# EnverRamirez/KiD

Hardware: AMD Instinct MI355X
Metric: thompson_mp_column_steps_per_sec (higher is better)
Workload: dtype f64; 1 GPU; config3: 100000 perturbed mixed-phase deep-convection columns, nz=120, dt=10 s, fp64; ncol_per_gpu=100000, nz=120

## Files before the change

### kid_amd/csrc/thompson_column.hip

```cpp
#include <hip/hip_runtime.h>

#include "thompson_column.h"
#include "fastmath.h"
#include "thompson_consts_gen.h"
#include "kernel_src_hash.h"

#include <cstdlib>
#include <type_traits>

#if defined(KIDMP_PROFILING)
#define DBGSTOP (a.debug_stop)
#define DBGCLK(var) const long long var = (DBGSTOP == 7 || DBGSTOP == 8) ? (long long)__builtin_readcyclecounter() : 0
#define PSTOP(code, expr)
#elif defined(KIDMP_PSTOP_AT)
#define DBGSTOP KIDMP_PSTOP_AT
#define DBGCLK(var)
#define PSTOP(code, expr) if (DBGSTOP == (code)) { L(V_QFAC, k) = (expr); break; }
#else
#define DBGSTOP 0
#define DBGCLK(var)
#define PSTOP(code, expr)
#endif

#ifndef KIDMP_REAL
// ... 374 lines not shown
            }
    }
}

__device__ inline real nr_from_mvd(real rr, real mvd)
{
    const dreal lamr = (R_(3.0) + mu_r + R_(0.672)) / Q(mvd);
    return real(R_(kc::crg[1]) * R_(kc::org3) * rr * cube(lamr) / am_r);
}

template <char SPECIES>
__device__ inline real eff_aero(real D, real Da, real visc, real rhoa, real Temp)
{
    const real boltzman = R_(1.3806503E-23), meanPath = R_(0.0256E-6);
    real vt;
    if constexpr (SPECIES == 'r')
        vt = -R_(0.1021) + R_(4.932E3) * D - R_(0.9551E6) * D * D + R_(0.07934E9) * D * D * D - R_(0.002362E12) * D * D * D * D;
    else if constexpr (SPECIES == 's')
        vt = av_s * fpow(D, bv_s);
    else
        vt = av_g * fpow(D, bv_g);
    const real Cc = R_(1.) + R_(2.) * meanPath / Q(Da) * (R_(1.257) + R_(0.4) * fm::exp(-R_(0.55) * Da / meanPath));
    const real diff = boltzman * Temp * Cc / Q((R_(3.) * PI * visc * Da));
    const real Re = R_(0.5) * rhoa * D * vt / Q(visc);
    const real Sc_ = visc / Q((rhoa * diff));
    const real St = Da * Da * vt * R_(1000.) / Q((R_(9.) * visc * D));
    const real aval = R_(1.) + fm::log(R_(1.) + Re);
    const real St2 = (R_(1.2) + R_(1.) / R_(12.) * aval) / Q((R_(1.) + aval));
    const real sRe = fm::sqrt_pos(Re);
    real Eff = R_(4.) / Q((Re * Sc_)) * (R_(1.) + R_(0.4) * sRe * fpow(Sc_, R_(0.3333)) + R_(0.16) * sRe * fm::sqrt_pos(Sc_))
             + R_(4.) * Da / Q(D) * (R_(0.02) + Da / Q(D) * (R_(1.) + R_(2.) * sRe));
    if (St > St2) {
        const real x = (St - St2) / Q((St - St2 + R_(0.666667)));
        Eff = Eff + x * fm::sqrt_pos(x);
    }
    return fmax(R_(1.E-5), fmin(Eff, R_(1.0)));
}
__device__ inline real ice_demott(real tempc, real rho, real nifa)
{
    const real rho_not0 = R_(101325.) / (R_(287.05) * R_(273.15));
    const real nifa_cc = nifa * rho_not0 * R_(1.E-6) / Q(rho);
    real xni = (R_(5.94e-5) * fpow(-tempc, R_(3.33))) * fpow(nifa_cc, ((-R_(0.0264) * (tempc)) + R_(0.0033)));
    xni = xni * rho / rho_not0 * R_(1000.);
    return fmax(R_(0.), xni);
}
__device__ inline real ice_koop(real temp, real qv, real qvs, real naero, real DT)
{
    const real R_uni = R_(8.314), ar_volume = R_(4.) / R_(3.) * PI * (R_(2.5e-6) * R_(2.5e-6) * R_(2.5e-6));
    const real satw = qv / Q(qvs);
    const real mu_diff = R_(210368.0) + (R_(131.438) * temp) - (R_(3.32373E6) / Q(temp)) - (R_(41729.1) * fm::log(temp));
    const real a_w_i = fm::exp(mu_diff / Q((R_uni * temp)));
    const real delta_aw = satw - a_w_i;
    real log_J_rate = -R_(906.7) + (R_(8502.0) * delta_aw) - (R_(26924.0) * delta_aw * delta_aw) + (R_(29180.0) * delta_aw * delta_aw * delta_aw);
    log_J_rate = fmin(R_(20.0), log_J_rate);
    const real J_rate = fm::exp10(fmax(log_J_rate, -R_(30.)));
    const real prob_h = fmin(R_(1.) - fm::exp(fmax(-J_rate * ar_volume * DT, -R_(80.))), R_(1.));
    real xni = R_(0.);
    if (prob_h > R_(0.)) xni = fmin(prob_h * naero, R_(1000.E3));
    return fmax(R_(0.0), xni);
}
__device__ inline real activ_ncloud(real Ww, real NCCN)
{
    const real ta_Na[7] = {R_(10.0), R_(31.6), R_(100.0), R_(316.0), R_(1000.0), R_(3160.0), R_(10000.0)};
    const real ta_Ww[9] = {R_(0.01), R_(0.0316), R_(0.1), R_(0.316), R_(1.0), R_(3.16), R_(10.0), R_(31.6), R_(100.0)};
    real n_local = NCCN * R_(1.E-6), w_local = Ww;
    if (n_local >= ta_Na[6]) n_local = ta_Na[6] - R_(1.0);
    else if (n_local <= ta_Na[0]) n_local = ta_Na[0] + R_(1.0);
    real xa = ta_Na[0], xb = ta_Na[1];
#pragma unroll
    for (int n = 1; n < 7; ++n) if (n_local >= ta_Na[n - 1] && n_local < ta_Na[n]) { xa = ta_Na[n - 1]; xb = ta_Na[n]; }
    if (w_local >= ta_Ww[8]) w_local = ta_Ww[8] - R_(1.0);
    else if (w_local <= ta_Ww[0]) w_local = ta_Ww[0] + R_(0.001);
    real ya = ta_Ww[0], yb = ta_Ww[1];
#pragma unroll
    for (int n = 1; n < 9; ++n) if (w_local >= ta_Ww[n - 1] && w_local < ta_Ww[n]) { ya = ta_Ww[n - 1]; yb = ta_Ww[n]; }
    const real x1 = fm::log(xa), x2 = fm::log(xb), y1 = fm::log(ya), y2 = fm::log(yb);
    const real nx = fm::log(n_local), wy = fm::log(w_local);
    const real t = (nx - x1) / Q((x2 - x1)), u = (wy - y1) / Q((y2 - y1));
    const real fraction = (R_(1.0) - t) * (R_(1.0) - u) * R_(1.0) + t * (R_(1.0) - u) * R_(1.0) + t * u * R_(1.0) + (R_(1.0) - t) * u * R_(1.0);
    return NCCN * fraction;
}

enum Slot {
    V_TEMP = 0, V_QV, V_RHO, V_RC, V_RI , V_RR, V_RS , V_RG , V_NI , V_NR, V_QVSI , V_SSATW,
    V_SSATI , V_N0X , V_PRES, V_NWFA , V_NIFA , V_NCRAW , V_NIRAW , V_NRRAW ,
    V_TTEN = 32 , V_QFAC, V_QCTEN , V_NCTEN , V_QITEN, V_NITEN, V_QRTEN, V_NRTEN, V_QSTEN, V_QGTEN,
    V_RHO2 , V_BOOST , V_RHOK , V_RR2, V_NR2, V_VTS0 ,
    V_MVDK ,
    NSLOT_V = 64,
    NSLOT_MIXED = 13,
    NSLOT_WARM = 10
};

enum Flag { F_QC = 1, F_QI = 2, F_QR = 4, F_QS = 8, F_QG = 16 };

struct SlotMap { int v[NSLOT_V]; };
constexpr SlotMap make_map(bool warm)
{
    SlotMap m{};
    for (int i = 0; i < NSLOT_V; ++i) m.v[i] = -1;
    if (warm) {
        m.v[V_TEMP] = 0; m.v[V_QV] = 1; m.v[V_RHO] = 2; m.v[V_RC] = 3; m.v[V_SSATW] = 4; m.v[V_RR] = 5; m.v[V_PRES] = 6; m.v[V_NR] = 7;
        m.v[V_QCTEN] = 0; m.v[V_NCTEN] = 1; m.v[V_QITEN] = 2; m.v[V_NITEN] = 3; m.v[V_QRTEN] = 4; m.v[V_NRTEN] = 5;
        m.v[V_QSTEN] = 6; m.v[V_QGTEN] = 7; m.v[V_RR2] = 8; m.v[V_NR2] = 9;
    } else {
        m.v[V_TEMP] = 0; m.v[V_QV] = 1; m.v[V_RHO] = 2; m.v[V_RC] = 3; m.v[V_RR] = 4; m.v[V_NI] = 5; m.v[V_NR] = 6;
        m.v[V_QVSI] = 7; m.v[V_SSATW] = 8; m.v[V_SSATI] = 9; m.v[V_N0X] = 10; m.v[V_PRES] = 11; m.v[V_RI] = 12;
        m.v[V_QFAC] = 0; m.v[V_QITEN] = 1; m.v[V_NITEN] = 2; m.v[V_QRTEN] = 3; m.v[V_NRTEN] = 4; m.v[V_QSTEN] = 5;
        m.v[V_QGTEN] = 6; m.v[V_BOOST] = 7; m.v[V_RHOK] = 8; m.v[V_RR2] = 9; m.v[V_MVDK] = 10; m.v[V_NR2] = 11; m.v[V_VTS0] = 12;
    }
    return m;
}
constexpr SlotMap WMAP = make_map(true), MMAP = make_map(false);
__device__ constexpr int mixed_slot(int v) { return MMAP.v[v]; }
template <bool WARM, int S>
__device__ constexpr int slot_of()
{
    static_assert(S >= 0 && S < NSLOT_V, "no such slot");
    static_assert((WARM ? WMAP.v[S] : MMAP.v[S]) >= 0, "this slot is not staged in this layout");
    return WARM ? WMAP.v[S] : MMAP.v[S];
}

}

__constant__ Consts g_consts[MAX_CONST_SLOTS];

typedef __attribute__((address_space(1))) real greal;
typedef __attribute__((address_space(1))) double grate;
__device__ inline greal *uniform_ptr(const real *p)
{
    const unsigned long long v = reinterpret_cast<unsigned long long>(p);
    const unsigned lo = __builtin_amdgcn_readfirstlane(unsigned(v));
    const unsigned hi = __builtin_amdgcn_readfirstlane(unsigned(v >> 32));
    return (greal *)((static_cast<unsigned long long>(hi) << 32) | lo);
}

__device__ inline greal *gptr(const real *p, int64_t off)
{
    return (greal *)reinterpret_cast<unsigned long long>(p) + off;
}
__device__ inline grate *gptr_rate(const double *p, int64_t off)
{
    return (grate *)reinterpret_cast<unsigned long long>(p) + off;
}

typedef const __attribute__((address_space(4))) StepArgs CArgs;
__device__ inline CArgs *kargs()
{
    CArgs *p = (CArgs *)__builtin_amdgcn_kernarg_segment_ptr();
    asm volatile("" : "+s"(p));
    return p;
}

#ifndef KIDMP_MIXED_WAVES
#define KIDMP_MIXED_WAVES 3
#endif
#ifndef KIDMP_WARM_WAVES
#define KIDMP_WARM_WAVES 4
#endif
#ifdef KIDMP_NUM_VGPR
#define KIDMP_VGPR_ATTR __attribute__((amdgpu_num_vgpr(KIDMP_NUM_VGPR)))
#else
#define KIDMP_VGPR_ATTR
#endif
template <int NJ, int NL, int CPW, bool RATES, bool WARM, bool AERO, bool NCCOL = false>
__global__ __launch_bounds__(CPW *WAVE, WARM ? KIDMP_WARM_WAVES : ((RATES || AERO) ? 2 : KIDMP_MIXED_WAVES)) KIDMP_VGPR_ATTR void thompson_column_step(const StepArgs a)
{
    constexpr int BL = WAVE / CPW;
    __shared__ dreal Lsh[CPW][(WARM ? NSLOT_WARM : NSLOT_MIXED) * NL];
    __shared__ int s_alive[CPW];
    __shared__ int s_next;
    __shared__ real s_cc[7][16];
    __shared__ double s_p10[P10_N];
    __shared__ real s_ntc[NCCOL && CPW > 1 ? CPW : 1];
    static_assert(!(NCCOL && AERO), "a per-column droplet number is for non-aerosol contexts");
    const int wv = CPW > 1 ? __builtin_amdgcn_readfirstlane(int(threadIdx.x) / WAVE) : 0;
    dreal *const Lw = Lsh[wv];
#define L(slot, k) Lw[slot_of<WARM, slot>() * NL + (k)]
#define LR(slot, k) Lw[mixed_slot(slot) * NL + (k)]

#if KFM_TABLES
    constexpr bool TABLES_AT_ENTRY = sizeof(dreal) == 8 && (!WARM || REAL_IS_BINARY32), TABLES_LATE = sizeof(dreal) == 8 && !TABLES_AT_ENTRY;
    if constexpr (TABLES_AT_ENTRY) {
        fm::tab::load_tables(int(threadIdx.x), CPW * WAVE);
        __syncthreads();
    }
    fm::tab::TableRequest<CPW * WAVE> mathtab;
    if constexpr (TABLES_LATE) mathtab.request(int(threadIdx.x));
#endif
    const Consts &c = g_consts[a.cslot];
    const int lane = lane_id();
    const int nz = a.nz;
    __builtin_assume(nz >= 2 && nz <= 4 * WAVE);
    const int kte = nz - 1;
    const unsigned nzu = unsigned(nz), kteu = unsigned(kte);
    constexpr bool iiwarm = WARM;
    const real DT = a.dt;
    const real odt = frcp(DT), odts = frcp(DT);
    real Nt_c = c.Nt_c;
    constexpr int NTAB = WARM ? 112 : 112 + P10_N;
    static_assert(P10_N == 32, "Consts::lds_tab holds 32 powers of ten");
    constexpr int TPT = (NTAB + CPW * WAVE - 1) / (CPW * WAVE);
    double tabv[TPT];
#pragma unroll
    for (int i = 0; i < TPT; ++i) {
        const int t = int(threadIdx.x) + i * CPW * WAVE;
        tabv[i] = c.lds_tab[t < NTAB ? t : 0];
    }

    const int64_t col0 = int64_t(blockIdx.x) * CPW;
    const int64_t col = col0 + wv;
    bool alive = col < a.ncol;
    if constexpr (NCCOL) {
        if (alive) {
            const unsigned long long pv = reinterpret_cast<unsigned long long>(kargs()->set_nc_col);
            const unsigned lo = __builtin_amdgcn_readfirstlane(unsigned(pv)), hi = __builtin_amdgcn_readfirstlane(unsigned(pv >> 32));
            typedef __attribute__((address_space(1))) double gdouble;
            Nt_c = real(((const gdouble *)((static_cast<unsigned long long>(hi) << 32) | lo))[col] * 1.e6);
        }
    }
    {
        if (DBGSTOP == 9) return;
        DBGCLK(clk0);
        const int64_t base = col * int64_t(nz), base0 = col0 * int64_t(nz);
        int pst[NJ];
        real mvdB[NJ], rgB[NJ];
        bool any_micro = false;
        bool col_frozen = true;
#pragma unroll
        for (int j = 0; j < NJ; ++j) { pst[j] = 0; mvdB[j] = R_(0.); rgB[j] = R1; }
        if (alive) {
        real i_t[NJ], i_qv[NJ], i_p[NJ], i_qc[NJ], i_qi[NJ], i_qr[NJ], i_qs[NJ], i_qg[NJ], i_ni[NJ], i_nr[NJ];
        real i_nc[NJ], i_nwfa[NJ], i_nifa[NJ];
        {
        CArgs *ka = kargs();
        const greal *gt = gptr(ka->t, base), *gqv = gptr(ka->qv, base), *gp = gptr(ka->p, base),
                      *gqc = gptr(ka->qc, base), *gqi = gptr(ka->qi, base), *gqr = gptr(ka->qr, base),
                      *gqs = gptr(ka->qs, base), *gqg = gptr(ka->qg, base), *gni = gptr(ka->ni, base),
                      *gnr = gptr(ka->nr, base), *gnc = gptr(ka->nc, base), *gnwfa = gptr(ka->nwfa, base),
                      *gnifa = gptr(ka->nifa, base);
#pragma unroll
        for (int j = 0; j < NJ; ++j) {
            const unsigned k = unsigned(lane) + unsigned(WAVE) * unsigned(j);
            const unsigned kc = k < nzu ? k : kteu;
            i_t[j] = gt[kc];   i_qv[j] = gqv[kc]; i_p[j] = gp[kc];   i_qc[j] = gqc[kc]; i_qi[j] = gqi[kc];
            i_qr[j] = gqr[kc]; i_qs[j] = gqs[kc]; i_qg[j] = gqg[kc]; i_ni[j] = gni[kc]; i_nr[j] = gnr[kc];
            i_nc[j] = gnc[kc]; i_nwfa[j] = gnwfa[kc]; i_nifa[j] = gnifa[kc];
        }
        }
        if constexpr (iiwarm) {
            bool fz = false;
#pragma unroll
            for (int j = 0; j < NJ; ++j) fz = fz || i_qi[j] != R_(0.) || i_qs[j] != R_(0.) || i_qg[j] != R_(0.) || i_ni[j] != R_(0.);
            col_frozen = __any(fz);
        }
#pragma unroll
        for (int j = 0; j < NJ; ++j) {
            const unsigned k = unsigned(lane) + unsigned(WAVE) * unsigned(j);
            pst[j] = 0; mvdB[j] = R_(0.); rgB[j] = R1;
            if (k >= nzu) continue;
            const real temp = i_t[j];
            const real qv = fmax(R_(1.E-10), i_qv[j]);
            const real pres = i_p[j];
            const real rho = R_(0.622) * pres / Q((Rgas * temp * (qv + R_(0.622))));
            const real qc1 = i_qc[j], qi1 = i_qi[j], qr1 = i_qr[j], qs1 = i_qs[j], qg1 = i_qg[j];
            int f = 0;
            real ri = R1, ni = R2, rr = R1, nr = R2, rg = R1;

            if (qc1 > R1) {
                f |= F_QC;
            }
            if (qi1 > R1) {
                f |= F_QI;
                ri = qi1 * rho;
                ni = fmax(R2, i_ni[j] * rho);
                if (ni <= R2) {
                    const dreal lami = R_(kc::cie[1]) / R_(25.E-6);
                    ni = fmin(R_(499.e3), R_(kc::cig[0]) * R_(kc::oig2) * ri / am_i * cube(lami));
                }
                dreal lami = root3(am_i * R_(kc::cig[1]) * R_(kc::oig1) * ni / Q(ri));
                const real xDi = (bm_i + mu_i + R_(1.)) * (frcp(lami));
                if (xDi < R_(5.E-6)) {
                    lami = R_(kc::cie[1]) / R_(5.E-6);
                    ni = fmin(R_(499.e3), R_(kc::cig[0]) * R_(kc::oig2) * ri / am_i * cube(lami));
                } else if (xDi > R_(300.E-6)) {
                    lami = R_(kc::cie[1]) / R_(300.E-6);
                    ni = R_(kc::cig[0]) * R_(kc::oig2) * ri / am_i * cube(lami);
                }
            }
            if (qr1 > R1) {
                f |= F_QR;
                rr = qr1 * rho;
                nr = fmax(R2, i_nr[j] * rho);
                if (nr <= R2) nr = nr_from_mvd(rr, R_(1.0E-3));
                const dreal lamr = root3(am_r * R_(kc::crg[2]) * R_(kc::org2) * nr / Q(rr));
                real mvd = (R_(3.0) + mu_r + R_(0.672)) / Q(lamr);
                if (mvd > R_(2.5E-3)) {
                    mvd = R_(2.5E-3);
                    nr = nr_from_mvd(rr, mvd);
                } else if (mvd < D0r * R_(0.75)) {
                    mvd = D0r * R_(0.75);
                    nr = nr_from_mvd(rr, mvd);
                }
                mvdB[j] = mvd;
            }
            if (qs1 > R1) f |= F_QS;
            if (qg1 > R1) { f |= F_QG; rg = qg1 * rho; }
            rgB[j] = rg;

            const real tempc = temp - R_(273.15);
            const real qvs = rslf(pres, temp);
            const real qvsi = tempc <= R_(0.0) ? rsif(pres, temp) : qvs;
            real ssatw = qv / Q(qvs) - R_(1.);
            real ssati = qv / Q(qvsi) - R_(1.);
            if (fabs(ssatw) < eps) ssatw = R_(0.0);
            if (fabs(ssati) < eps) ssati = R_(0.0);
            if (f != 0 || ssati > R_(0.0)) any_micro = true;
            pst[j] = f | (temp >= R_(270.65) ? 1 << 16 : 0);

            L(V_TEMP, k) = temp;  L(V_QV, k) = i_qv[j];   L(V_RHO, k) = rho;
            L(V_RC, k) = (f & F_QC) ? qc1 : R_(0.);  L(V_RR, k) = (f & F_QR) ? qr1 : R_(0.);
            L(V_NR, k) = nr;      L(V_SSATW, k) = ssatw;
            L(V_PRES, k) = pres;
            if constexpr (!iiwarm) {
                L(V_RI, k) = (f & F_QI) ? qi1 : R_(0.);
                L(V_NI, k) = ni;      L(V_QVSI, k) = qvsi;  L(V_SSATI, k) = ssati;
            }
        }

        if (!__any(any_micro)) {
            CArgs *ka = kargs();
            greal *gqc = gptr(ka->qc, base), *gnc = gptr(ka->nc, base), *gqi = gptr(ka->qi, base),
                    *gni = gptr(ka->ni, base), *gqr = gptr(ka->qr, base), *gnr = gptr(ka->nr, base),
                    *gqs = gptr(ka->qs, base), *gqg = gptr(ka->qg, base);
            grate *grates = RATES ? gptr_rate(ka->rates, col * int64_t(KIDMP_NRATES_) * nz) : nullptr;
#pragma unroll
            for (int j = 0; j < NJ; ++j) {
                const unsigned k = unsigned(lane) + unsigned(WAVE) * unsigned(j);
                if (k >= nzu) continue;
                gqc[k] = R_(0.0); gnc[k] = R_(0.0);
                gqr[k] = R_(0.0); gnr[k] = R_(0.0);
                if (col_frozen) { gqi[k] = R_(0.0); gni[k] = R_(0.0); gqs[k] = R_(0.0); gqg[k] = R_(0.0); }
                if (RATES)
                    for (int r = 0; r < KIDMP_NRATES_; ++r) grates[int64_t(r) * nz + k] = R_(0.);
            }
            if (ka->nstep && lane < 4) ka->nstep[col * 4 + lane] = 0;
            alive = false;
        }

        if constexpr (!iiwarm) if (alive) {
            int k0l = 0;
#pragma unroll
            for (int j = 0; j < NJ; ++j)
                if (pst[j] >> 16) k0l = lane + WAVE * j;
            const int k_0 = wave_max_i(k0l);
            dreal n0[NJ];
            bool in_[NJ], ur_[NJ];
#pragma unroll
            for (int j = 0; j < NJ; ++j) {
                const unsigned k = unsigned(lane) + unsigned(WAVE) * unsigned(j);
                in_[j] = k < nzu;
                ur_[j] = int(k) > k_0 && (pst[j] & F_QR) && mvdB[j] > R_(100.E-6);
            }
            graupel_N0_column<NJ>(in_, ur_, mvdB, rgB, dreal(c.n0g_empty), n0);
            suffix_min<NJ>(n0);
#pragma unroll
            for (int j = 0; j < NJ; ++j) {
                const unsigned k = unsigned(lane) + unsigned(WAVE) * unsigned(j);
                if (k < nzu) L(V_N0X, k) = n0[j];
            }
        }

        }
        if (DBGSTOP == 1) { if (alive && lane == 0) kargs()->ppt[col * 4] += Lw[0] + Lw[9 * NL + 1]; return; }
#pragma unroll
        for (int i = 0; i < TPT; ++i) {
            const int t = int(threadIdx.x) + i * CPW * WAVE;
            if (t < 112) s_cc[t >> 4][t & 15] = real(tabv[i]);
            else if (!WARM && t < NTAB) s_p10[t - 112] = tabv[i];
        }
#if KFM_TABLES
        if constexpr (TABLES_LATE) mathtab.store(int(threadIdx.x));
#endif
        DBGCLK(clk1);
        if (CPW > 1) {
            if (lane == 0) s_alive[wv] = alive ? (col_frozen ? 3 : 1) : 0;
            if (threadIdx.x == 0) s_next = 0;
            if constexpr (NCCOL) if (lane == 0) s_ntc[wv] = Nt_c;
            __syncthreads();
        }
        DBGCLK(clk2);
        if (CPW == 1 && !alive) return;
#undef L
#define L(slot, k) Lp[slot_of<WARM, slot>() * NL + (k)]
        const int nband = (nz + BL - 1) / BL;
#pragma unroll 1
        for (int it = 0;; ++it) {
            int seq = it;
            if (CPW > 1) {
                int t = 0;
                if (lane == 0) t = atomicAdd(&s_next, 1);
                seq = __builtin_amdgcn_readfirstlane(t);
            }
            if (seq >= nband) break;
            const int band = CPW > 1 ? (nband - 1) / 2 + ((seq & 1) ? (seq + 1) / 2 : -(seq / 2)) : seq;
            const int cw = CPW > 1 ? lane / BL : 0;
            const unsigned k = unsigned(band * BL) + unsigned(lane % BL);
            if (k < nzu && (CPW == 1 || s_alive[cw])) do {
            dreal *const Lp = Lsh[cw];
            if constexpr (NCCOL && CPW > 1) Nt_c = s_ntc[cw];
            const unsigned gk = unsigned(cw) * nzu + k;
            CArgs *ka1 = kargs();
            real qi1c, qs1c, qg1c, ni_b = R2, ni1_raw, qvsi = R_(0.), ssati = R_(0.), diffu = R_(0.);
            const bool frozen_here = !iiwarm || (CPW == 1 ? col_frozen : (s_alive[cw] & 2) != 0);
            if constexpr (iiwarm) {
                qi1c = R_(0.); qs1c = R_(0.); qg1c = R_(0.); ni1_raw = R_(0.);
                if (frozen_here) {
                    const real rqi = gptr(ka1->qi, base0)[gk], rqs = gptr(ka1->qs, base0)[gk], rqg = gptr(ka1->qg, base0)[gk];
                    ni1_raw = gptr(ka1->ni, base0)[gk];
                    qi1c = rqi > R1 ? rqi : R_(0.);  qs1c = rqs > R1 ? rqs : R_(0.);  qg1c = rqg > R1 ? rqg : R_(0.);
                }
            } else {
                const real rqs = gptr(ka1->qs, base0)[gk], rqg = gptr(ka1->qg, base0)[gk];
                qi1c = L(V_RI, k);  qs1c = rqs > R1 ? rqs : R_(0.);  qg1c = rqg > R1 ? rqg : R_(0.);
                ni_b = L(V_NI, k);
                qvsi = L(V_QVSI, k);  ssati = L(V_SSATI, k);
            }
            real nwfa_in = R_(0.), nifa_in = R_(0.), nc_in = R_(0.), nr_in = R_(0.);
            if constexpr (AERO) {
                nwfa_in = gptr(ka1->nwfa, base0)[gk]; nifa_in = gptr(ka1->nifa, base0)[gk];
                nc_in = gptr(ka1->nc, base0)[gk];     nr_in = gptr(ka1->nr, base0)[gk];
                if constexpr (!iiwarm) ni1_raw = gptr(ka1->ni, base0)[gk];
            }
            const bool L_qc = L(V_RC, k) > R_(0.), L_qi = qi1c > R_(0.), L_qr = L(V_RR, k) > R_(0.), L_qs = qs1c > R_(0.), L_qg = qg1c > R_(0.);
            const real pres = L(V_PRES, k);
            grate *grates = RATES ? gptr_rate(ka1->rates, col0 * int64_t(KIDMP_NRATES_) * nz) + int64_t(cw) * KIDMP_NRATES_ * nz : nullptr;
            const real temp = L(V_TEMP, k), qv_raw = L(V_QV, k), rho = L(V_RHO, k);
            const real qv = fmax(R_(1.E-10), qv_raw);
            const real rc = L_qc ? L(V_RC, k) * rho : R1, ri = L_qi ? qi1c * rho : R1,
                         rr = L_qr ? L(V_RR, k) * rho : R1;
            const real rs = L_qs ? qs1c * rho : R1, rg = L_qg ? qg1c * rho : R1;
            const real ni = ni_b, nr = L(V_NR, k);
            const real ssatw = L(V_SSATW, k);
            real nc = L_qc ? Nt_c : R_(2.);
            real nwfa_k = R_(0.), nifa_k = R_(0.);
            if constexpr (AERO) {
                nwfa_k = fmax(R_(11.1E6), fmin(R_(9999.E6), nwfa_in * rho));
                nifa_k = fmax(naIN1 * R_(0.01), fmin(R_(9999.E6), nifa_in * rho));
                if (L_qc) {
                    nc = fmax(R_(2.), nc_in * rho);
                    int nu = int(lround(R_(1000.E6) / Q(nc))) + 2;
                    nu = nu < 15 ? nu : 15;
                    dreal lc = root3(nc * am_r * s_cc[1][nu - 1] * s_cc[2][nu - 1] / Q(rc));
                    const real xD = (bm_r + nu + R_(1.)) / Q(lc);
                    if (xD < D0c)                lc = s_cc[4][nu - 1] / D0c;
                    else if (xD > D0r * R_(2.))  lc = s_cc[4][nu - 1] / (D0r * R_(2.));
                    nc = fmin(dreal(Nt_c_max), s_cc[0][nu - 1] * s_cc[3][nu - 1] * rc / am_r * cube(lc));
                }
            }

            const real tempc = temp - R_(273.15);
            const real rhof = fm::sqrt_pos(rho_not / Q(rho));
            const real rhof2 = fm::sqrt_pos(rhof);
            const real visco = visc_air(tempc);
            const real vsc2 = fm::sqrt_pos(rho / Q(visco));
            const real tcond = (R_(5.69) + R_(0.0168) * tempc) * R_(1.0E-5) * R_(418.936);

            dreal lamr = R_(1.), N0_r = R_(0.);
            real mvd_r = R_(0.);
            if (L_qr) {
                lamr = root3(am_r * R_(kc::crg[2]) * R_(kc::org2) * nr / Q(rr));
                mvd_r = (R_(3.0) + mu_r + R_(0.672)) / Q(lamr);
                N0_r = nr * R_(kc::org2) * lamr;
            }

            dreal pnc_wau = 0, pnc_rcw = 0, pnc_scw = 0, pnc_gcw = 0;
            dreal prr_wau = 0, prr_rcw = 0, prr_rcs = 0, prr_rcg = 0, prr_sml = 0, prr_gml = 0, prr_rci = 0;
            dreal pnr_wau = 0, pnr_rcs = 0, pnr_rcg = 0, pnr_rci = 0, pnr_sml = 0, pnr_gml = 0, pnr_rcr = 0, pnr_rfz = 0;
            dreal pri_inu = 0, pni_inu = 0, pri_ihm = 0, pni_ihm = 0, pri_wfz = 0, pni_wfz = 0, pri_rfz = 0,
                   pni_rfz = 0, pri_ide = 0, pni_ide = 0, pri_rci = 0, pni_rci = 0, pni_sci = 0, pni_iau = 0;
            dreal pri_iha = 0, pni_iha = 0;
            dreal na_m = R_(0.), nd_m = R_(0.);
            dreal prs_iau = 0, prs_sci = 0, prs_rcs = 0, prs_scw = 0, prs_sde = 0, prs_ihm = 0, prs_ide = 0;
            dreal prg_scw = 0, prg_rfz = 0, prg_gde = 0, prg_gcw = 0, prg_rci = 0, prg_rcs = 0, prg_rcg = 0, prg_ihm = 0;
            real vts_boost = R_(1.5);
            dreal nc_m = R_(0.), ni_p = R_(0.), ni_m = R_(0.), nr_p = R_(0.), nr_m = R_(0.);

            if (L_qr && mvd_r > D0r) {
                const real Ef_rr = R_(1.0) - fm::exp(R_(2300.0) * (mvd_r - R_(1950.0E-6)));
                pnr_rcr = Ef_rr * R_(2.0) * nr * rr;
                nr_m += pnr_rcr;
            }
            real mvd_c = D0c;
            int nu_c = 15;
            dreal lamc = R_(1.);
            real xDc = R_(0.);
            if (L_qc) {
                nu_c = int(lround(R_(1000.E6) / Q(nc))) + 2;
                nu_c = nu_c < 15 ? nu_c : 15;
                lamc = root3(nc * am_r * s_cc[1][nu_c - 1] * s_cc[2][nu_c - 1] / Q(rc));
                if constexpr (sizeof(real) == 8) xDc = fmax(D0c * R_(1.E6), (s_cc[6][nu_c - 1] / Q(lamc)) * R_(1.E6));
                else                             xDc = fmax(D0c * R_(1.E6), root3(rc / Q((am_r * nc))) * R_(1.E6));
                mvd_c = (R_(3.0) + nu_c + R_(0.672)) / Q(lamc);
            }
            if (rc > R_(0.01e-3)) {
                const real Dc_g = (s_cc[5][nu_c - 1] / Q(lamc)) * R_(1.E6);
                const real Dc_b = root6(xDc * xDc * xDc * Dc_g * Dc_g * Dc_g - xDc * xDc * xDc * xDc * xDc * xDc);
                const real zq = R_(6.25E-6) * xDc * Dc_b * Dc_b * Dc_b - R_(0.4);
                const real zeta1 = R_(0.5) * (zq + fabs(zq));
                const real zeta = R_(0.027) * rc * zeta1;
                const real tq = R_(0.5) * Dc_b - R_(7.5);
                const real taud = R_(0.5) * (tq + fabs(tq)) + R1;
                const real tau = R_(3.72) / Q((rc * taud));
                prr_wau = zeta / Q(tau);
                prr_wau = fmin(rc * odts, prr_wau);
                pnr_wau = prr_wau / Q((am_r * nu_c * D0r * D0r * D0r));
                pnc_wau = fmin(nc * odts, prr_wau / Q((am_r * mvd_c * mvd_c * mvd_c)));
                nr_p += pnr_wau;
                nc_m += pnc_wau;
            }
            if (L_qr && mvd_r > D0r && mvd_c > D0c) {
                int idx = 1 + int(nbins * fm::log(mvd_r / R_(kc::Dr1)) / R_(kc::log_Drn_Dr1));
                idx = idx < nbins ? idx : nbins;
                idx = idx > 1 ? idx : 1;
                int jc = int(mvd_c * R_(1.E6));
                jc = jc < 1 ? 1 : (jc > nbins ? nbins : jc);
                const real Ef_rw = kargs()->tables.t_Efrw[(idx - 1) + nbins * (jc - 1)];
                const dreal coll = frcp(pw4(lamr + fv_r));
                prr_rcw = rhof * R_(kc::t1_qr_qc) * Ef_rw * rc * N0_r * coll;
                prr_rcw = fmin(rc * odts, prr_rcw);
                pnc_rcw = rhof * R_(kc::t1_qr_qc) * Ef_rw * nc * N0_r * coll;
                pnc_rcw = fmin(nc * odts, pnc_rcw);
                nc_m += pnc_rcw;
            }
            if constexpr (AERO) if (L_qr && mvd_r > D0r) {
                const dreal coll = frcp(pw4(lamr + fv_r));
                real Ef_ra = eff_aero<'r'>(mvd_r, R_(0.04E-6), visco, rho, temp);
                dreal pna_rca = rhof * R_(kc::t1_qr_qc) * Ef_ra * nwfa_k * N0_r * coll;
                pna_rca = fmin(dreal(nwfa_k * odts), pna_rca);
                Ef_ra = eff_aero<'r'>(mvd_r, R_(0.8E-6), visco, rho, temp);
                dreal pnd_rcd = rhof * R_(kc::t1_qr_qc) * Ef_ra * nifa_k * N0_r * coll;
                pnd_rcd = fmin(dreal(nifa_k * odts), pnd_rcd);
                na_m += pna_rca;
                nd_m += pnd_rcd;
            }

            real smob = R_(0.), smo0 = R_(0.), smo1 = R_(0.), smoc = R_(0.), smoe = R_(0.), smof = R_(0.);
            if constexpr (!iiwarm) if (L_qs) {
                const real tc0 = fmin(-R_(0.1), temp - R_(273.15));
                smob = rs * R_(kc::oams);
                const Log2Parts lsmo2 = log2_parts(smob);
                if constexpr (KIDMP_FIT_CUBIC && sizeof(real) == 8) {
                    smo0 = snow_moment_c<-2>(lsmo2, tc0);
                    smo1 = snow_moment_c<-1>(lsmo2, tc0);
                } else {
                {
                    const real la = R_(kc::sa[0]) + R_(kc::sa[1]) * tc0 + R_(kc::sa[4]) * tc0 * tc0 + R_(kc::sa[8]) * tc0 * tc0 * tc0;
                    const real b_ = R_(kc::sb[0]) + R_(kc::sb[1]) * tc0 + R_(kc::sb[4]) * tc0 * tc0 + R_(kc::sb[8]) * tc0 * tc0 * tc0;
                    smo0 = pow10_times_pow(la, lsmo2, b_);
                }
                {
                    const real la = R_(kc::sa[0]) + R_(kc::sa[1]) * tc0 + R_(kc::sa[2]) + R_(kc::sa[3]) * tc0 + R_(kc::sa[4]) * tc0 * tc0 + R_(kc::sa[5])
                                    + R_(kc::sa[6]) * tc0 * tc0 + R_(kc::sa[7]) * tc0 + R_(kc::sa[8]) * tc0 * tc0 * tc0 + R_(kc::sa[9]);
                    const real b_ = R_(kc::sb[0]) + R_(kc::sb[1]) * tc0 + R_(kc::sb[2]) + R_(kc::sb[3]) * tc0 + R_(kc::sb[4]) * tc0 * tc0 + R_(kc::sb[5])
                                    + R_(kc::sb[6]) * tc0 * tc0 + R_(kc::sb[7]) * tc0 + R_(kc::sb[8]) * tc0 * tc0 * tc0 + R_(kc::sb[9]);
                    smo1 = pow10_times_pow(la, lsmo2, b_);
                }
                }
                smoc = snow_moment_c<0>(lsmo2, tc0);
                smoe = snow_moment_c<12>(lsmo2, tc0);
                smof = snow_moment_c<15>(lsmo2, tc0);
            }

            PSTOP(21, smob + smo0 + smo1 + smoc + smoe + smof + rhof + rhof2 + vsc2 + tcond)
            dreal ilamg = R_(0.), N0_g = R_(0.), ig_bv = R_(0.), ig11 = R_(0.), lamg_E = R_(1.);
            if constexpr (!iiwarm) if (L_qg) {
                const dreal N0_exp = L(V_N0X, k);
                const dreal lam_exp = root4(N0_exp * am_g * R_(kc::cgg[0]) / Q(rg));
                const dreal lamg = lam_exp * R_(kc::lamg_fac);
                lamg_E = lamg;
                ilamg = frcp(lamg);
                N0_g = N0_exp / Q((R_(kc::cgg[1]) * lam_exp)) * lamg;
                ig_bv = fpow(ilamg, bv_g);
                ig11 = ilamg * ilamg * fm::sqrt_pos(ilamg * ig_bv);
            }

            PSTOP(22, smob + smo0 + smo1 + smoc + smoe + smof + rhof + rhof2 + vsc2 + tcond + ilamg + N0_g + ig_bv + ig11 + lamg_E
                          + lamr + N0_r + mvd_r + pnr_rcr + prr_wau + pnr_wau + pnc_wau + prr_rcw + pnc_rcw + nc_m + nr_p + nr_m
                          + na_m + nd_m + mvd_c + lamc + xDc + dreal(nu_c))
            if (!iiwarm) {
                int idx_tc = int(lround(-tempc));
                idx_tc = idx_tc < 45 ? idx_tc : 45;
                idx_tc = idx_tc > 1 ? idx_tc : 1;
                int idx_t = int((tempc - R_(2.5)) / R_(5.)) - 1;
                idx_t = 1 > -idx_t ? 1 : -idx_t;
                idx_t = idx_t < ntb_t ? idx_t : ntb_t;

                const int idx_c = rc > R_(kc::r_c1) ? decade_idx(rc, kc::nic2, ntb_c, s_p10) : 1;
                const int idx_i = ri > R_(kc::r_i1) ? decade_idx(ri, kc::nii2, ntb_i, s_p10) : 1;
                const int idx_i1 = ni > R_(kc::Nt_i1) ? decade_idx(ni, kc::nii3, ntb_i1, s_p10) : 1;
                int idx_r = 1, idx_r1 = ntb_r1;
                if (rr > R_(kc::r_r1)) {
                    idx_r = decade_idx(rr, kc::nir2, ntb_r, s_p10);
                    const dreal lam_exp = lamr * R_(kc::lamr_exp_fac);
                    const dreal N0_exp = R_(kc::org1) * rr / am_r * pw4(lam_exp);
                    idx_r1 = decade_idx(N0_exp, kc::nir3, ntb_r1, s_p10);
                }
                const int idx_s = rs > R_(kc::r_s1) ? decade_idx(rs, kc::nis2, ntb_s, s_p10) : 1;
                int idx_g = 1, idx_g1 = ntb_g1;
                if (rg > R_(kc::r_g1)) {
                    idx_g = decade_idx(rg, kc::nig2, ntb_g, s_p10);
                    const dreal lamg = lamg_E;
                    const dreal lam_exp = lamg * R_(kc::lamg_exp_fac);
                    const dreal N0_exp = R_(kc::ogg1) * rg / am_g * pw4(lam_exp);
                    idx_g1 = decade_idx(N0_exp, kc::nig3, ntb_g1, s_p10);
                }

                real rvs = R_(0.), t1_subl = R_(0.);
                if (L_qi || L_qs || L_qg) {
                    diffu = diffusivity(temp, pres);
                    const real otemp = frcp(temp);
                    rvs = rho * qvsi;
                    const real h1 = otemp * (lsub * otemp * oRv - R_(1.));
                    const real rvs_p = rvs * otemp * (lsub * otemp * oRv - R_(1.));
                    const real rvs_pp = rvs * (h1 * h1 + (-R_(2.) * lsub * otemp * otemp * otemp * oRv) + otemp * otemp);
                    const real gamsc = lsub * diffu / Q(tcond) * rvs_p;
                    real alphsc = R_(0.5) * (gamsc / Q((R_(1.) + gamsc))) * (gamsc / Q((R_(1.) + gamsc))) * rvs_pp / Q(rvs_p) * rvs / Q(rvs_p);
                    alphsc = fmax(R_(1.E-9), alphsc);
                    real xsat = ssati;
                    if (fabs(xsat) < R_(1.E-9)) xsat = R_(0.);
                    t1_subl = R_(4.) * PI * (R_(1.0) - alphsc * xsat + R_(2.) * alphsc * alphsc * xsat * xsat
                                             - R_(5.) * alphsc * alphsc * alphsc * xsat * xsat * xsat) / Q((R_(1.) + gamsc));
                }

                if (L_qc && mvd_c > D0c) {
                    const real xDs = L_qs ? smoc / Q(smob) : R_(0.0);
                    int jc = int(mvd_c * R_(1.E6));
                    jc = jc < 1 ? 1 : (jc > nbins ? nbins : jc);
                    if (xDs > D0s) {
                        int idx = 1 + int(nbins * fm::log(xDs / R_(kc::Ds1)) / R_(kc::log_Dsn_Ds1));
                        idx = idx < nbins ? idx : nbins;
                        idx = idx > 1 ? idx : 1;
                        const real Ef_sw = kargs()->tables.t_Efsw[(idx - 1) + nbins * (jc - 1)];
                        prs_scw = rhof * R_(kc::t1_qs_qc) * Ef_sw * rc * smoe;
                        pnc_scw = rhof * R_(kc::t1_qs_qc) * Ef_sw * nc * smoe;
                        pnc_scw = fmin(nc * odts, pnc_scw);
                        nc_m += pnc_scw;
                    }
                    if (rg >= R_(kc::r_g1) && mvd_c > D0c) {
                        const real xDg = (bm_g + mu_g + R_(1.)) * ilamg;
                        const real vtg = rhof * av_g * R_(kc::cgg[5]) * R_(kc::ogg3) * ig_bv;
                        const real stoke_g = mvd_c * mvd_c * vtg * rho_w / Q((R_(9.) * visco * xDg));
                        if (xDg > D0g) {
                            real Ef_gw = R_(0.);
                            if (stoke_g >= R_(0.4) && stoke_g <= R_(10.)) Ef_gw = R_(0.55) * fm::log10(R_(2.51) * stoke_g);
                            else if (stoke_g < R_(0.4))               Ef_gw = R_(0.0);
                            else if (stoke_g > 10)                Ef_gw = R_(0.77);
                            const dreal ig9 = cube(ilamg) * ig_bv;
                            prg_gcw = rhof * R_(kc::t1_qg_qc) * Ef_gw * rc * N0_g * ig9;
                            pnc_gcw = rhof * R_(kc::t1_qg_qc) * Ef_gw * nc * N0_g * ig9;
                            pnc_gcw = fmin(nc * odts, pnc_gcw);
                            nc_m += pnc_gcw;
                        }
                    }
                }

                if constexpr (AERO) {
                    if (rs > R_(kc::r_s1)) {
                        const real xDs = smoc / Q(smob);
                        real Ef_sa = eff_aero<'s'>(xDs, R_(0.04E-6), visco, rho, temp);
                        dreal pna_sca = rhof * R_(kc::t1_qs_qc) * Ef_sa * nwfa_k * smoe;
                        pna_sca = fmin(dreal(nwfa_k * odts), pna_sca);
                        Ef_sa = eff_aero<'s'>(xDs, R_(0.8E-6), visco, rho, temp);
                        dreal pnd_scd = rhof * R_(kc::t1_qs_qc) * Ef_sa * nifa_k * smoe;
                        pnd_scd = fmin(dreal(nifa_k * odts), pnd_scd);
                        na_m += pna_sca;
                        nd_m += pnd_scd;
                    }
                    if (rg > R_(kc::r_g1)) {
                        const real xDg = (bm_g + mu_g + R_(1.)) * ilamg;
                        const dreal ig9 = cube(ilamg) * ig_bv;
                        real Ef_ga = eff_aero<'g'>(xDg, R_(0.04E-6), visco, rho, temp);
                        dreal pna_gca = rhof * R_(kc::t1_qg_qc) * Ef_ga * nwfa_k * N0_g * ig9;
                        pna_gca = fmin(dreal(nwfa_k * odts), pna_gca);
                        Ef_ga = eff_aero<'g'>(xDg, R_(0.8E-6), visco, rho, temp);
                        dreal pnd_gcd = rhof * R_(kc::t1_qg_qc) * Ef_ga * nifa_k * N0_g * ig9;
                        pnd_gcd = fmin(dreal(nifa_k * odts), pnd_gcd);
                        na_m += pna_gca;
                        nd_m += pnd_gcd;
                    }
                }

                if (rr >= R_(kc::r_r1)) {
                    if (rs >= R_(kc::r_s1)) {
                        const int64_t id = (idx_s - 1) + int64_t(ntb_s) * ((idx_t - 1) + int64_t(ntb_t) * ((idx_r1 - 1) + int64_t(ntb_r1) * (idx_r - 1)));
                        const double *r = kargs()->tables.racs_rec + id * RACS_REC;
                        const dreal tmr_racs1 = r[0], tcr_sacr1 = r[1], tmr_racs2 = r[2], tcr_sacr2 = r[3],
                                     tcs_racs1 = r[4], tms_sacr1 = r[5];
                        if (temp < T_0) {
                            prr_rcs = -(tmr_racs2 + tcr_sacr2 + tmr_racs1 + tcr_sacr1);
                            prs_rcs = tmr_racs2 + tcr_sacr2 - tcs_racs1 - tms_sacr1;
                            prg_rcs = tmr_racs1 + tcr_sacr1 + tcs_racs1 + tms_sacr1;
                            prr_rcs = fmax(-rr * odts, prr_rcs);
                            prs_rcs = fmax(-rs * odts, prs_rcs);
                            prg_rcs = fmin((rr + rs) * odts, prg_rcs);
                            pnr_rcs = r[6] + r[7] + r[8] + r[9];
                        } else {
                            prs_rcs = -tcs_racs1 - tms_sacr1 + tmr_racs2 + tcr_sacr2;
                            prs_rcs = fmax(-rs * odts, prs_rcs);
                            prr_rcs = -prs_rcs;
                            pnr_rcs = r[7] + r[9];
                        }
                        pnr_rcs = fmin(nr * odts, pnr_rcs);
                        nr_m += pnr_rcs;
                    }
                    if (rg >= R_(kc::r_g1)) {
                        const int64_t id = (idx_g1 - 1) + int64_t(ntb_g1) * ((idx_g - 1) + int64_t(ntb_g) * ((idx_r1 - 1) + int64_t(ntb_r1) * (idx_r - 1)));
                        const double *r = kargs()->tables.racg_rec + id * RACG_REC;
                        if (temp < T_0) {
                            prg_rcg = r[0] + r[1];
                            prg_rcg = fmin(rr * odts, prg_rcg);
                            prr_rcg = -prg_rcg;
                            pnr_rcg = r[2] + r[3];
                            pnr_rcg = fmin(nr * odts, pnr_rcg);
                        } else {
                            prr_rcg = r[4];
                            prr_rcg = fmin(rg * odts, prr_rcg);
                            prg_rcg = -prr_rcg;
                            pnr_rcg = -R_(5.) * r[3];
                        }
                        nr_m += pnr_rcg;
                    }
                }

                if (temp < T_0) {
                    vts_boost = R_(1.0);
                    const real rate_max = (qv - qvsi) * rho * odts * R_(0.999);

                    if (rr > R_(kc::r_r1)) {
                        const int64_t id = (idx_r - 1) + int64_t(ntb_r) * ((idx_r1 - 1) + int64_t(ntb_r1) * (idx_tc - 1));
                        const double *r = kargs()->tables.qrfz_rec + id * QRFZ_REC;
                        prg_rfz = r[0] * odts;
                        pri_rfz = r[1] * odts;
                        pni_rfz = r[2] * odts;
                        pnr_rfz = r[3] * odts;
                        pnr_rfz = fmin(nr * odts, pnr_rfz);
                        nr_m += pnr_rfz;
                        ni_p += pni_rfz;
                    } else if (rr > R1 && temp < HGFR) {
                        pri_rfz = rr * odts;
                        pnr_rfz = nr * odts;
                        pni_rfz = pnr_rfz;
                        nr_m += pnr_rfz;
                        ni_p += pni_rfz;
                    }
                    if (rc > R_(kc::r_c1)) {
                        const int id = (idx_c - 1) + ntb_c * (idx_tc - 1);
                        pri_wfz = kargs()->tables.tpi_qcfz[id] * odts;
                        pri_wfz = fmin(rc * odts, pri_wfz);
                        pni_wfz = kargs()->tables.tni_qcfz[id] * odts;
                        pni_wfz = fmin(fmin(Nt_c * odts, pri_wfz / Q((R_(2.) * xm0i))), pni_wfz);
                        nc_m += pni_wfz;
                        ni_p += pni_wfz;
                    } else if (rc > R1 && temp < HGFR) {
                        pri_wfz = rc * odts;
                        pni_wfz = nc * odts;
                        nc_m += pni_wfz;
                        ni_p += pni_wfz;
                    }

                    if ((ssati >= R_(0.25)) || (ssatw > eps && temp < R_(253.15))) {
                        real xnc;
                        if constexpr (AERO) xnc = ice_demott(tempc, rho, nifa_k);
                        else                xnc = fmin(R_(250.E3), TNO * fm::exp(ATO * (T_0 - temp)));
                        const real xni = ni + (pni_rfz + pni_wfz) * DT;
                        pni_inu = R_(0.5) * (xnc - xni + fabs(xnc - xni)) * odts;
                        pri_inu = fmin(rate_max, xm0i * pni_inu);
                        pni_inu = pri_inu / Q(xm0i);
                        ni_p += pni_inu;
                    }
                    if constexpr (AERO) {
                        const real xni = smo0 + ni + (pni_rfz + pni_wfz + pni_inu) * DT;
                        if ((xni <= R_(500.E3)) && (temp < R_(238.)) && (ssati >= R_(0.4))) {
                            const real xnc = ice_koop(temp, qv, rslf(pres, temp), nwfa_k, DT);
                            pni_iha = xnc * odts;
                            pri_iha = fmin(dreal(rate_max), xm0i * R_(0.1) * pni_iha);
                            pni_iha = pri_iha / Q((xm0i * R_(0.1)));
                        }
                    }

                    if (L_qi) {
                        const dreal lami = root3(am_i * R_(kc::cig[1]) * R_(kc::oig1) * ni / Q(ri));
                        const dreal ilami = frcp(lami);
                        const real xDi = fmax(dreal(R_(kc::D0i)), (bm_i + mu_i + R_(1.)) * ilami);
                        const real xmi = am_i * cube(xDi);
                        const real oxmi = frcp(xmi);
                        pri_ide = C_cube * t1_subl * diffu * ssati * rvs * R_(kc::oig1) * R_(kc::cig[4]) * ni * ilami;
                        const int id = (idx_i - 1) + ntb_i * (idx_i1 - 1);
                        if (pri_ide < R_(0.0)) {
                            pri_ide = fmax(fmax(-ri * odts, pri_ide), rate_max);
                            pni_ide = pri_ide * oxmi;
                            pni_ide = fmax(-ni * odts, pni_ide);
                        } else {
                            pri_ide = fmin(pri_ide, rate_max);
                            const dreal frac = kargs()->tables.tpi_ide[id];
                            prs_ide = (R_(1.0) - frac) * pri_ide;
                            pri_ide = frac * pri_ide;
                        }
                        if ((idx_i == ntb_i) || (xDi > R_(5.0) * D0s)) {
                            prs_iau = ri * R_(.99) * odts;
                            pni_iau = ni * R_(.95) * odts;
                        } else if (xDi < R_(0.1) * D0s) {
                            prs_iau = R_(0.);
                            pni_iau = R_(0.);
                        } else {
                            prs_iau = kargs()->tables.tps_iaus[id] * odts;
                            prs_iau = fmin(ri * R_(.99) * odts, prs_iau);
                            pni_iau = kargs()->tables.tni_iaus[id] * odts;
                            pni_iau = fmin(ni * R_(.95) * odts, pni_iau);
                        }
                        ni_m += pni_iau;
                        if (rs >= R_(kc::r_s1)) {
                            prs_sci = R_(kc::t1_qs_qi) * rhof * Ef_si * ri * smoe;
                            pni_sci = prs_sci * oxmi;
                            ni_m += pni_sci;
                        }
                        if (rr >= R_(kc::r_r1) && mvd_r > R_(4.) * xDi) {
                            const dreal c9 = frcp(pw4(lamr + fv_r));
                            pri_rci = rhof * R_(kc::t1_qr_qi) * Ef_ri * ri * N0_r * c9;
                            pnr_rci = rhof * R_(kc::t1_qr_qi) * Ef_ri * ni * N0_r * c9;
                            pni_rci = pri_rci * oxmi;
                            ni_m += pni_rci;
                            nr_m += pnr_rci;
                            prr_rci = rhof * R_(kc::t2_qr_qi) * Ef_ri * ni * N0_r * (frcp(pw7(lamr + fv_r)));
                            prr_rci = fmin(rr * odts, prr_rci);
                            prg_rci = pri_rci + prr_rci;
                        }
                    }

                    if (L_qs) {
                        real C_snow = C_sqrd + (tempc + R_(1.5)) * (C_cube - C_sqrd) / Q((-R_(30.) + R_(1.5)));
                        C_snow = fmax(C_sqrd, fmin(C_snow, C_cube));
                        prs_sde = C_snow * t1_subl * diffu * ssati * rvs * (R_(kc::t1_qs_sd) * smo1 + R_(kc::t2_qs_sd) * rhof2 * vsc2 * smof);
                        if (prs_sde < R_(0.)) prs_sde = fmax(fmax(-rs * odts, prs_sde), rate_max);
                        else              prs_sde = fmin(prs_sde, rate_max);
                    }
                    if (L_qg && ssati < -eps) {
                        prg_gde = C_cube * t1_subl * diffu * ssati * rvs * N0_g
                                * (R_(kc::t1_qg_sd) * (ilamg * ilamg) + R_(kc::t2_qg_sd) * vsc2 * rhof2 * ig11);
                        if (prg_gde < R_(0.)) prg_gde = fmax(fmax(-rg * odts, prg_gde), rate_max);
                        else              prg_gde = fmin(prg_gde, rate_max);
                    }

                    if (prg_gcw > eps && tempc > -R_(8.0)) {
                        real tf = R_(0.);
                        if (tempc >= -R_(5.0) && tempc < -R_(3.0))      tf = R_(0.5) * (-R_(3.0) - tempc);
                        else if (tempc > -R_(8.0) && tempc < -R_(5.0))  tf = R_(0.33333333) * (R_(8.0) + tempc);
                        pni_ihm = R_(3.5E8) * tf * prg_gcw;
                        pri_ihm = xm0i * pni_ihm;
                        ni_p += pni_ihm;
                        prs_ihm = prs_scw / Q((prs_scw + prg_gcw)) * pri_ihm;
                        prg_ihm = prg_gcw / Q((prs_scw + prg_gcw)) * pri_ihm;
                    }
                    if (prs_scw > R_(2.0) * prs_sde && prs_sde > eps) {
                        const real r_frac = fmin(R_(30.0), prs_scw / Q(prs_sde));
                        const real g_frac = fmin(R_(0.95), R_(0.15) + (r_frac - R_(2.)) * R_(.028));
                        vts_boost = fmin(R_(1.5), R_(1.1) + (r_frac - R_(2.)) * R_(.016));
                        prg_scw = g_frac * prs_scw;
                        prs_scw = (R_(1.) - g_frac) * prs_scw;
                    }
                } else {
                    const real delQvs = fmax(R_(0.0), rslf(pres, R_(273.15)) - qv);
                    if (L_qs) {
                        prr_sml = (tempc * tcond - lvap0 * diffu * delQvs) * (R_(kc::t1_qs_me) * smo1 + R_(kc::t2_qs_me) * rhof2 * vsc2 * smof);
                        prr_sml = prr_sml + R_(4218.) * olfus * tempc * (prr_rcs + prs_scw);
                        prr_sml = fmin(rs * odts, fmax(R_(0.), prr_sml));
                        pnr_sml = smo0 / Q(rs) * prr_sml * fm::exp10(-R_(0.25) * tempc);
                        pnr_sml = fmin(smo0 * odts, pnr_sml);
                        nr_p += pnr_sml;
                        if (ssati < R_(0.)) {
// ... 1140 lines not shown
```

Measured before the change: 73.85 million column-steps/s.

## Defer ice number diagnosis to cold branch and cache rain slope in LDS

Moves the ice number/slope (ni, lami) diagnosis out of the staging pass into the sub-freezing branch of the rates pass, where it is the only place it is used. The ice number is read from global memory there, or earlier, instead of being staged in a local slot. The rain slope lamr is computed once at staging, recomputed after clamping, and stored in the freed slot so the rates pass need not repeat the cube root. This removes redundant cube roots and skips ice work at warm levels, at the cost of an extra global load and some code motion that could shift register pressure.

```diff
diff --git a/kid_amd/csrc/thompson_column.hip b/kid_amd/csrc/thompson_column.hip
--- a/kid_amd/csrc/thompson_column.hip
+++ b/kid_amd/csrc/thompson_column.hip
@@ -480,7 +480,7 @@
 }
 
 enum Slot {
-    V_TEMP = 0, V_QV, V_RHO, V_RC, V_RI , V_RR, V_RS , V_RG , V_NI , V_NR, V_QVSI , V_SSATW,
+    V_TEMP = 0, V_QV, V_RHO, V_RC, V_RI , V_RR, V_RS , V_RG , V_LAMR, V_NR, V_QVSI , V_SSATW,
     V_SSATI , V_N0X , V_PRES, V_NWFA , V_NIFA , V_NCRAW , V_NIRAW , V_NRRAW ,
     V_TTEN = 32 , V_QFAC, V_QCTEN , V_NCTEN , V_QITEN, V_NITEN, V_QRTEN, V_NRTEN, V_QSTEN, V_QGTEN,
     V_RHO2 , V_BOOST , V_RHOK , V_RR2, V_NR2, V_VTS0 ,
@@ -499,10 +499,11 @@
     for (int i = 0; i < NSLOT_V; ++i) m.v[i] = -1;
     if (warm) {
         m.v[V_TEMP] = 0; m.v[V_QV] = 1; m.v[V_RHO] = 2; m.v[V_RC] = 3; m.v[V_SSATW] = 4; m.v[V_RR] = 5; m.v[V_PRES] = 6; m.v[V_NR] = 7;
+        m.v[V_LAMR] = 8;
         m.v[V_QCTEN] = 0; m.v[V_NCTEN] = 1; m.v[V_QITEN] = 2; m.v[V_NITEN] = 3; m.v[V_QRTEN] = 4; m.v[V_NRTEN] = 5;
         m.v[V_QSTEN] = 6; m.v[V_QGTEN] = 7; m.v[V_RR2] = 8; m.v[V_NR2] = 9;
     } else {
-        m.v[V_TEMP] = 0; m.v[V_QV] = 1; m.v[V_RHO] = 2; m.v[V_RC] = 3; m.v[V_RR] = 4; m.v[V_NI] = 5; m.v[V_NR] = 6;
+        m.v[V_TEMP] = 0; m.v[V_QV] = 1; m.v[V_RHO] = 2; m.v[V_RC] = 3; m.v[V_RR] = 4; m.v[V_LAMR] = 5; m.v[V_NR] = 6;
         m.v[V_QVSI] = 7; m.v[V_SSATW] = 8; m.v[V_SSATI] = 9; m.v[V_N0X] = 10; m.v[V_PRES] = 11; m.v[V_RI] = 12;
         m.v[V_QFAC] = 0; m.v[V_QITEN] = 1; m.v[V_NITEN] = 2; m.v[V_QRTEN] = 3; m.v[V_NRTEN] = 4; m.v[V_QSTEN] = 5;
         m.v[V_QGTEN] = 6; m.v[V_BOOST] = 7; m.v[V_RHOK] = 8; m.v[V_RR2] = 9; m.v[V_MVDK] = 10; m.v[V_NR2] = 11; m.v[V_VTS0] = 12;
@@ -663,44 +664,26 @@
             const real rho = R_(0.622) * pres / Q((Rgas * temp * (qv + R_(0.622))));
             const real qc1 = i_qc[j], qi1 = i_qi[j], qr1 = i_qr[j], qs1 = i_qs[j], qg1 = i_qg[j];
             int f = 0;
-            real ri = R1, ni = R2, rr = R1, nr = R2, rg = R1;
+            real rr = R1, nr = R2, rg = R1;
 
             if (qc1 > R1) {
                 f |= F_QC;
             }
-            if (qi1 > R1) {
-                f |= F_QI;
-                ri = qi1 * rho;
-                ni = fmax(R2, i_ni[j] * rho);
-                if (ni <= R2) {
-                    const dreal lami = R_(kc::cie[1]) / R_(25.E-6);
-                    ni = fmin(R_(499.e3), R_(kc::cig[0]) * R_(kc::oig2) * ri / am_i * cube(lami));
-                }
-                dreal lami = root3(am_i * R_(kc::cig[1]) * R_(kc::oig1) * ni / Q(ri));
-                const real xDi = (bm_i + mu_i + R_(1.)) * (frcp(lami));
-                if (xDi < R_(5.E-6)) {
-                    lami = R_(kc::cie[1]) / R_(5.E-6);
-                    ni = fmin(R_(499.e3), R_(kc::cig[0]) * R_(kc::oig2) * ri / am_i * cube(lami));
-                } else if (xDi > R_(300.E-6)) {
-                    lami = R_(kc::cie[1]) / R_(300.E-6);
-                    ni = R_(kc::cig[0]) * R_(kc::oig2) * ri / am_i * cube(lami);
-                }
-            }
+            if (qi1 > R1) f |= F_QI;
             if (qr1 > R1) {
                 f |= F_QR;
                 rr = qr1 * rho;
                 nr = fmax(R2, i_nr[j] * rho);
                 if (nr <= R2) nr = nr_from_mvd(rr, R_(1.0E-3));
-                const dreal lamr = root3(am_r * R_(kc::crg[2]) * R_(kc::org2) * nr / Q(rr));
+                dreal lamr = root3(am_r * R_(kc::crg[2]) * R_(kc::org2) * nr / Q(rr));
                 real mvd = (R_(3.0) + mu_r + R_(0.672)) / Q(lamr);
-                if (mvd > R_(2.5E-3)) {
-                    mvd = R_(2.5E-3);
+                if (mvd > R_(2.5E-3) || mvd < D0r * R_(0.75)) {
+                    mvd = mvd > R_(2.5E-3) ? R_(2.5E-3) : D0r * R_(0.75);
                     nr = nr_from_mvd(rr, mvd);
-                } else if (mvd < D0r * R_(0.75)) {
-                    mvd = D0r * R_(0.75);
-                    nr = nr_from_mvd(rr, mvd);
+                    lamr = root3(am_r * R_(kc::crg[2]) * R_(kc::org2) * nr / Q(rr));
                 }
                 mvdB[j] = mvd;
+                L(V_LAMR, k) = lamr;
             }
             if (qs1 > R1) f |= F_QS;
             if (qg1 > R1) { f |= F_QG; rg = qg1 * rho; }
@@ -722,7 +705,7 @@
             L(V_PRES, k) = pres;
             if constexpr (!iiwarm) {
                 L(V_RI, k) = (f & F_QI) ? qi1 : R_(0.);
-                L(V_NI, k) = ni;      L(V_QVSI, k) = qvsi;  L(V_SSATI, k) = ssati;
+                L(V_QVSI, k) = qvsi;  L(V_SSATI, k) = ssati;
             }
         }
 
@@ -809,7 +792,8 @@
             if constexpr (NCCOL && CPW > 1) Nt_c = s_ntc[cw];
             const unsigned gk = unsigned(cw) * nzu + k;
             CArgs *ka1 = kargs();
-            real qi1c, qs1c, qg1c, ni_b = R2, ni1_raw, qvsi = R_(0.), ssati = R_(0.), diffu = R_(0.);
+            constexpr bool NI_LATE = RATES && CPW == 1 && sizeof(dreal) == 4;
+            real qi1c, qs1c, qg1c, ni_rawB = R_(0.), ni1_raw, qvsi = R_(0.), ssati = R_(0.), diffu = R_(0.);
             const bool frozen_here = !iiwarm || (CPW == 1 ? col_frozen : (s_alive[cw] & 2) != 0);
             if constexpr (iiwarm) {
                 qi1c = R_(0.); qs1c = R_(0.); qg1c = R_(0.); ni1_raw = R_(0.);
@@ -821,14 +805,14 @@
             } else {
                 const real rqs = gptr(ka1->qs, base0)[gk], rqg = gptr(ka1->qg, base0)[gk];
                 qi1c = L(V_RI, k);  qs1c = rqs > R1 ? rqs : R_(0.);  qg1c = rqg > R1 ? rqg : R_(0.);
-                ni_b = L(V_NI, k);
+                if constexpr (!AERO && !NI_LATE) ni_rawB = gptr(ka1->ni, base0)[gk];
                 qvsi = L(V_QVSI, k);  ssati = L(V_SSATI, k);
             }
             real nwfa_in = R_(0.), nifa_in = R_(0.), nc_in = R_(0.), nr_in = R_(0.);
             if constexpr (AERO) {
                 nwfa_in = gptr(ka1->nwfa, base0)[gk]; nifa_in = gptr(ka1->nifa, base0)[gk];
                 nc_in = gptr(ka1->nc, base0)[gk];     nr_in = gptr(ka1->nr, base0)[gk];
-                if constexpr (!iiwarm) ni1_raw = gptr(ka1->ni, base0)[gk];
+                if constexpr (!iiwarm) { ni1_raw = gptr(ka1->ni, base0)[gk]; ni_rawB = ni1_raw; }
             }
             const bool L_qc = L(V_RC, k) > R_(0.), L_qi = qi1c > R_(0.), L_qr = L(V_RR, k) > R_(0.), L_qs = qs1c > R_(0.), L_qg = qg1c > R_(0.);
             const real pres = L(V_PRES, k);
@@ -838,7 +822,7 @@
             const real rc = L_qc ? L(V_RC, k) * rho : R1, ri = L_qi ? qi1c * rho : R1,
                          rr = L_qr ? L(V_RR, k) * rho : R1;
             const real rs = L_qs ? qs1c * rho : R1, rg = L_qg ? qg1c * rho : R1;
-            const real ni = ni_b, nr = L(V_NR, k);
+            const real nr = L(V_NR, k);
             const real ssatw = L(V_SSATW, k);
             real nc = L_qc ? Nt_c : R_(2.);
             real nwfa_k = R_(0.), nifa_k = R_(0.);
@@ -867,7 +851,7 @@
             dreal lamr = R_(1.), N0_r = R_(0.);
             real mvd_r = R_(0.);
             if (L_qr) {
-                lamr = root3(am_r * R_(kc::crg[2]) * R_(kc::org2) * nr / Q(rr));
+                lamr = L(V_LAMR, k);
                 mvd_r = (R_(3.0) + mu_r + R_(0.672)) / Q(lamr);
                 N0_r = nr * R_(kc::org2) * lamr;
             }
@@ -996,7 +980,6 @@
 
                 const int idx_c = rc > R_(kc::r_c1) ? decade_idx(rc, kc::nic2, ntb_c, s_p10) : 1;
                 const int idx_i = ri > R_(kc::r_i1) ? decade_idx(ri, kc::nii2, ntb_i, s_p10) : 1;
-                const int idx_i1 = ni > R_(kc::Nt_i1) ? decade_idx(ni, kc::nii3, ntb_i1, s_p10) : 1;
                 int idx_r = 1, idx_r1 = ntb_r1;
                 if (rr > R_(kc::r_r1)) {
                     idx_r = decade_idx(rr, kc::nir2, ntb_r, s_p10);
@@ -1134,6 +1117,7 @@
                 if (temp < T_0) {
                     vts_boost = R_(1.0);
                     const real rate_max = (qv - qvsi) * rho * odts * R_(0.999);
+                    if constexpr (!AERO && NI_LATE) ni_rawB = gptr(kargs()->ni, base0)[gk];
 
                     if (rr > R_(kc::r_r1)) {
                         const int64_t id = (idx_r - 1) + int64_t(ntb_r) * ((idx_r1 - 1) + int64_t(ntb_r1) * (idx_tc - 1));
@@ -1167,6 +1151,28 @@
                         ni_p += pni_wfz;
                     }
 
+                    real ni = R2;
+                    dreal ilami = R_(0.);
+                    if (L_qi) {
+                        ni = fmax(R2, ni_rawB * rho);
+                        if (ni <= R2) {
+                            const dreal lami = R_(kc::cie[1]) / R_(25.E-6);
+                            ni = fmin(R_(499.e3), R_(kc::cig[0]) * R_(kc::oig2) * ri / am_i * cube(lami));
+                        }
+                        dreal lami = root3(am_i * R_(kc::cig[1]) * R_(kc::oig1) * ni / Q(ri));
+                        ilami = frcp(lami);
+                        const real xDi = (bm_i + mu_i + R_(1.)) * ilami;
+                        if (xDi < R_(5.E-6)) {
+                            lami = R_(kc::cie[1]) / R_(5.E-6);
+                            ni = fmin(R_(499.e3), R_(kc::cig[0]) * R_(kc::oig2) * ri / am_i * cube(lami));
+                            ilami = frcp(root3(am_i * R_(kc::cig[1]) * R_(kc::oig1) * ni / Q(ri)));
+                        } else if (xDi > R_(300.E-6)) {
+                            lami = R_(kc::cie[1]) / R_(300.E-6);
+                            ni = R_(kc::cig[0]) * R_(kc::oig2) * ri / am_i * cube(lami);
+                            ilami = frcp(root3(am_i * R_(kc::cig[1]) * R_(kc::oig1) * ni / Q(ri)));
+                        }
+                    }
+
                     if ((ssati >= R_(0.25)) || (ssatw > eps && temp < R_(253.15))) {
                         real xnc;
                         if constexpr (AERO) xnc = ice_demott(tempc, rho, nifa_k);
@@ -1188,12 +1194,11 @@
                     }
 
                     if (L_qi) {
-                        const dreal lami = root3(am_i * R_(kc::cig[1]) * R_(kc::oig1) * ni / Q(ri));
-                        const dreal ilami = frcp(lami);
                         const real xDi = fmax(dreal(R_(kc::D0i)), (bm_i + mu_i + R_(1.)) * ilami);
                         const real xmi = am_i * cube(xDi);
                         const real oxmi = frcp(xmi);
                         pri_ide = C_cube * t1_subl * diffu * ssati * rvs * R_(kc::oig1) * R_(kc::cig[4]) * ni * ilami;
+                        const int idx_i1 = ni > R_(kc::Nt_i1) ? decade_idx(ni, kc::nii3, ntb_i1, s_p10) : 1;
                         const int id = (idx_i - 1) + ntb_i * (idx_i1 - 1);
                         if (pri_ide < R_(0.0)) {
                             pri_ide = fmax(fmax(-ri * odts, pri_ide), rate_max);
```

Measured after the change: 74.57 million column-steps/s (median of 6 runs). About the same (+1.0%).
